# swarth100/dynfu

Hardware: AMD Instinct MI355X
Metric: frames/sec (warp-solve + TSDF fuse), 512^3 vol / 2k nodes / VGA depth (higher is better)
Workload: dtype f32; 1 GPU; C2: 512^3 TSDF, 640x480 depth, 2048 nodes, k=4, 262144 vertices, 5 GN x PCG<=256 (tol 1e-6), reference-parity energy (energy.t), lambda=200; parallelism=replicas x1 (one sequence per GPU, no collective), ranks_seen=1, repeats=5

## Files before the change

dynfu_amd/csrc/capi.cpp:

```cpp
#include <hip/hip_runtime.h>

#include <cmath>
#include <cstdarg>
#include <cstdio>
#include <cstring>
#include <map>
#include <mutex>
#include <new>
#include <utility>
#include <vector>

#include "../../include/dynfu_amd.h"
#include "kernels.hpp"
#include "dev_switch.hpp"
#include "solve.hpp"
#include "solve6.hpp"

namespace {

thread_local char g_err[512] = "";

int fail(int code, const char* fmt, ...) {
    va_list ap;
    va_start(ap, fmt);
// ... 87 lines not shown
    long cap_segs       = 0;
    hipError_t reserve(long nsegs) {
        if (nsegs <= cap_segs) return hipSuccess;
        (void)hipFree(seg_off), (void)hipFree(chunk_sums);
        seg_off = chunk_sums = nullptr, cap_segs = 0;
        hipError_t e;
        if ((e = hipMalloc((void**)&seg_off, sizeof(int32_t) * (size_t)(nsegs + 1))) != hipSuccess) return e;
        if ((e = hipMalloc((void**)&chunk_sums, sizeof(int32_t) * (size_t)dfa::mc_scan_chunks(nsegs))) != hipSuccess)
            return e;
        cap_segs = nsegs;
        return hipSuccess;
    }
};
struct McIndexedScratch {
    McScratch vert;
    int32_t* idx_off = nullptr;
    long cap_segs    = 0;
    hipError_t reserve(long nsegs) {
        hipError_t e = vert.reserve(nsegs);
        if (e != hipSuccess || nsegs <= cap_segs) return e;
        (void)hipFree(idx_off);
        idx_off = nullptr, cap_segs = 0;
        if ((e = hipMalloc((void**)&idx_off, sizeof(int32_t) * (size_t)(nsegs + 1))) != hipSuccess) return e;
        cap_segs = nsegs;
        return hipSuccess;
    }
};

bool want_grid(int D, long n_query) { return D >= 64 && ((long)D * n_query >= (1L << 22) || D >= 1024); }

}

struct dfa_solver {
    int max_D, max_N, k;
    size_t max_R;
    int ell_cap;
    dfa::SolveView v;
    dfa::SolveState* state;
    double* cost_partials;
    unsigned int* ticket;
    std::vector<void*> blocks;
    GridScratch grid;
    bool has_problem;
    bool timing;
    std::vector<hipEvent_t> events;
    std::vector<int> ev_pcg, ev_asm;
    size_t ev_used;
    int timed_solves = 0;
    dfa::MbGraphCache mb_graphs;
    dfa::TeamPcg team;
    bool deterministic = false;
    bool just_reset = false;
    bool graph_rows = false;
    long long* iters_total = nullptr;
    dfa_overlap_fn overlap_fn = nullptr;
    void* overlap_user        = nullptr;
    int* host_flag = nullptr;
};

struct dfa_solver6 {
    int max_D, max_N, k;
    dfa::Solve6View v;
    dfa::Solve6State* state;
    float* raw_w;
    int32_t* raw_reg;
    const float* node_dq;
    std::vector<void*> blocks;
    GridScratch grid;
    bool has_problem;
    std::map<int, hipGraphExec_t> pcg_graphs;
    int last_launches = 0;
    static constexpr int S6_RING = 4;
    int* mirror = nullptr;
    hipEvent_t done_ev[S6_RING] = {};
    int slot_gn[S6_RING] = {};
    unsigned long long solve_seq = 0, folded = 0;
    int pred[dfa::S6_HIST] = {};
    struct BudgetKey { int D, N, num_iter, gn_iter, linear_iter; float tol, tol_first, tol_decay, tol_adapt, gn_tol; } budget_key = {};
    bool graph_disabled = false;
    hipStream_t capture_stream = nullptr;
    bool timing = false;
    std::vector<hipEvent_t> events;
    size_t ev_used = 0;
    int pcg_key_D = -1;
};

namespace {
template <class T>
int plan6_alloc(dfa_solver6* s, T** out, size_t count) {
    void* p      = nullptr;
    hipError_t e = hipMalloc(&p, sizeof(T) * (count ? count : 1));
    if (e != hipSuccess) return hip_fail(e, "hipMalloc (solver6 plan)");
    s->blocks.push_back(p);
    *out = (T*)p;
    return DFA_OK;
}
}

namespace {
int timing_begin(dfa_solver* s, hipStream_t st) {
    if (s->ev_used + 2 > s->events.size()) {
        for (int i = 0; i < 2; ++i) {
            hipEvent_t e;
            if (hipEventCreate(&e) != hipSuccess) return -1;
            s->events.push_back(e);
        }
// ... 610 lines not shown
                                   out_normals, out_index, grid, S(stream)));
    return DFA_OK;
}

int dfa_correspond_projective(const float* vertices, const float* normals, int n, const float* vmap, int vmap_step,
                              const float* nmap, int nmap_step, int cols, int rows, float fx, float fy, float cx, float cy,
                              float dist_thresh, float min_cosine, float* out_vertices, float* out_normals,
                              int32_t* out_pixel, dfa_stream_t stream) {
    REQUIRE(n >= 0 && (n == 0 || vertices), "bad vertices");
    REQUIRE(vmap && cols > 0 && rows > 0 && vmap_step >= 16 * cols, "bad vertex map");
    REQUIRE(!nmap || nmap_step >= 16 * cols, "bad normal map pitch");
    REQUIRE(!out_normals || nmap, "normals requested without a normal map");
    REQUIRE(fx > 0.f && fy > 0.f && dist_thresh >= 0.f, "bad intrinsics / threshold");
    REQUIRE(((uintptr_t)vmap & 15) == 0 && (vmap_step & 15) == 0 && ((uintptr_t)nmap & 15) == 0 && (!nmap || (nmap_step & 15) == 0),
            "maps must be 16-byte aligned float4 images");
    HIP_TRY(dfa::launch_correspond_projective(vertices, normals, n, vmap, vmap_step, nmap, nmap_step, cols, rows, fx, fy, cx,
                                              cy, dist_thresh, min_cosine, out_vertices, out_normals, out_pixel,
                                              S(stream)));
    return DFA_OK;
}


int dfa_solver_create(int max_D, int max_N, int k, dfa_solver** out) {
    REQUIRE(out, "null out");
    *out = nullptr;
    REQUIRE(max_D > 0 && max_N >= 0, "bad sizes");
    REQUIRE(k >= 1 && k <= DFA_MAX_KNN, "k out of range 1..16");
    REQUIRE(max_D <= dfa::solve_pcg_max_nodes(), "more nodes than a plan supports (32768)");
    int ndev = 0;
    if (hipGetDeviceCount(&ndev) != hipSuccess || ndev == 0) return fail(DFA_ERR_NO_GPU, "no HIP device");
    dfa_solver* s = new (std::nothrow) dfa_solver();
    REQUIRE(s, "out of host memory");
    s->max_D = max_D, s->max_N = max_N, s->k = k;
    s->max_R       = (size_t)max_N + (size_t)max_D * k;
    s->ell_cap     = 256;
    s->has_problem = false;
    s->timing      = false;
    {
        const char* e    = getenv("DFA_ASSEMBLE_DETERMINISTIC");
        s->deterministic = e && atoi(e) != 0;
    }
    s->ev_used     = 0;
    std::memset(&s->v, 0, sizeof(s->v));
    const size_t R = s->max_R, D = (size_t)max_D;
    int rc = DFA_OK;
#define A(field, count) \
    if (rc == DFA_OK) rc = plan_alloc(s, &s->v.field, (count))
    A(ridx, R * k);
    A(rw, R * k);
    A(rtau, R);
    A(rb, R * 3);
    A(re, R * (size_t)dfa::solve_rec_words(k));
    A(reg_idx, D * k);
    A(blk_hist, D * (dfa::SOLVE_TG_BLOCKS + 1));
    A(node_ptr, D + 1);
    A(node_list, R * k);
    A(ell, D * s->ell_cap);
    A(ell_cnt, D);
    A(diag, D);
    A(g, D * 3);
    A(g_base, D * 3);
    A(t_base, D * 3);
    A(pk_perm, D);
    A(pk_perm2, D);
    A(pk_vals, D * s->ell_cap);
    A(pk_cols, D * s->ell_cap);
    A(mb_x, D);
    A(mb_r, D);
    A(mb_p, D);
    A(mb_s, D);
    A(mb_w, D);
    A(mb_u[0], D);
    A(mb_u[1], D);
    A(mb_m[0], D);
    A(mb_m[1], D);
    A(mb_t[0], D);
    A(mb_t[1], D);
    A(mb_gpart[0], (size_t)dfa::solve_mb_blocks(max_D));
    A(mb_gpart[1], (size_t)dfa::solve_mb_blocks(max_D));
    A(mb_dpart[0], (size_t)dfa::solve_mb_blocks(max_D));
    A(mb_dpart[1], (size_t)dfa::solve_mb_blocks(max_D));
    A(t, D * 3);
    A(huber, D);
    A(node_dq_out, D * 8);
#undef A
    if (rc == DFA_OK) {
        hipError_t e = s->grid.reserve(max_D);
        if (e != hipSuccess) rc = hip_fail(e, "hipMalloc (node grid)");
    }
    if (rc == DFA_OK && dfa::solve_team_pcg_fits(max_D) && (max_D > 2048 || dfa::kDevAB)) {
        s->v.team_stride = (max_D + 3) & ~3;
        rc = plan_alloc(s, &s->v.team_ctl, 1);
        const size_t areas = (size_t)3 * dfa::solve_team_pcg_rounds();
        if (rc == DFA_OK) rc = plan_alloc(s, &s->v.team_mt, areas * s->v.team_stride);
        if (rc == DFA_OK) rc = plan_alloc(s, &s->v.team_words, dfa::solve_team_pcg_words());
        if (rc == DFA_OK && (hipMemset(s->v.team_ctl, 0, sizeof(dfa::TeamCtl)) != hipSuccess ||
                             hipMemset(s->v.team_words, 0, sizeof(unsigned long long) * dfa::solve_team_pcg_words()) != hipSuccess ||
                             hipMemset(s->v.team_mt, 0, sizeof(float2) * areas * (size_t)s->v.team_stride) != hipSuccess))
            rc = fail(DFA_ERR_HIP, "hipMemset (team PCG)");
        if (rc == DFA_OK && hipHostMalloc((void**)&s->team.host_abort, sizeof(int), hipHostMallocDefault) == hipSuccess) {
            *s->team.host_abort = 0;
            s->team.ctl = s->v.team_ctl;
            if (const char* e0 = dfa::dev_env("DFA_MB_TEAM_EPOCH")) s->team.epoch = (unsigned)std::strtoul(e0, nullptr, 0);
        }
    }
    if (rc == DFA_OK) rc = plan_alloc(s, &s->state, 1);
    if (rc == DFA_OK) rc = plan_alloc(s, &s->iters_total, 1);
    if (rc == DFA_OK && hipMemset(s->iters_total, 0, sizeof(long long)) != hipSuccess) rc = DFA_ERR_HIP;
    if (rc == DFA_OK && hipHostMalloc((void**)&s->host_flag, 4 * sizeof(int), hipHostMallocDefault) != hipSuccess) s->host_flag = nullptr;
    if (rc == DFA_OK) rc = plan_alloc(s, &s->cost_partials, std::max<size_t>((R + 255) / 256 + 1, 1024) + 1024);
    if (rc == DFA_OK) rc = plan_alloc(s, &s->ticket, 64);
    if (rc == DFA_OK && hipMemset(s->ticket, 0, 64 * sizeof(unsigned int)) != hipSuccess)
        rc = fail(DFA_ERR_HIP, "hipMemset (ticket)");
    if (rc != DFA_OK) {
        dfa_solver_destroy(s);
        return rc;
    }
    *out = s;
    return DFA_OK;
}

void dfa_solver_destroy(dfa_solver* s) {
    if (!s) return;
    for (void* p : s->blocks) (void)hipFree(p);
    s->grid.release();
    for (hipEvent_t e : s->events) (void)hipEventDestroy(e);
    if (s->host_flag) (void)hipHostFree(s->host_flag);
    if (s->team.host_abort) (void)hipHostFree(s->team.host_abort);
    s->mb_graphs.release();
    delete s;
}

int dfa_solver_set_problem(dfa_solver* s, const float* node_pos, const float* node_dq, const float* node_w, int D,
                           const float* canon_vertices, const float* canon_normals, const float* live_vertices,
                           const float* live_normals, int N, dfa_stream_t stream) {
    (void)canon_normals;
    (void)live_normals;
    REQUIRE(s, "null plan");
    REQUIRE(node_pos && node_dq && node_w && D > 0, "no nodes");
    REQUIRE(N >= 0 && (N == 0 || (canon_vertices && live_vertices)), "bad vertex arrays");
    if (D > s->max_D || N > s->max_N)
        return fail(DFA_ERR_CAPACITY, "dfa_solver_set_problem: D=%d N=%d exceed the plan (max_D=%d max_N=%d)", D, N,
                    s->max_D, s->max_N);
    dfa::SolveView& v = s->v;
    v.N = N, v.D = D, v.k = s->k, v.Dpad = (D + 3) & ~3, v.ell_cap = s->ell_cap;
    v.deterministic = s->deterministic ? 1 : 0;
    v.node_pos = node_pos, v.node_dq = node_dq, v.node_w = node_w;
    v.canon = canon_vertices, v.live = live_vertices;
    hipStream_t st = S(stream);
    const dfa::KnnGridView* grid = nullptr;
    if (want_grid(D, (long)N + D) || dfa::dev_env_int("DFA_GRAPH_GRID", 0) != 0) {
        HIP_TRY(dfa::knn_grid_build(s->grid.v, node_pos, D, st));
        grid = &s->grid.v;
    }
    s->graph_rows = grid && dfa::solve_graph_rows_fits(v);
    if (s->graph_rows) {
        HIP_TRY(dfa::solve_build_graph_rows(v, *grid, s->state, s->ticket, 64, st));
    } else {
        if (N > 0) HIP_TRY(dfa::launch_knn(node_pos, node_w, D, canon_vertices, N, s->k, v.ridx, v.rw, grid, st));
        HIP_TRY(dfa::launch_knn(node_pos, node_w, D, node_pos, D, s->k, v.reg_idx, nullptr, grid, st));
        HIP_TRY(dfa::solve_build_graph(v, s->state, s->ticket, 64, st));
    }
    s->has_problem = true;
    s->just_reset  = true;
    return DFA_OK;
}

int dfa_solver_set_deterministic(dfa_solver* s, int on) {
    REQUIRE(s, "null plan");
    s->deterministic = on != 0;
    return DFA_OK;
}

int dfa_solver_solve(dfa_solver* s, const dfa_solve_params* p, dfa_stream_t stream) {
    REQUIRE(s && p, "null plan / params");
    REQUIRE(s->has_problem, "set_problem has not been called");
    REQUIRE(p->num_iter >= 0 && p->nonlinear_iter >= 0 && p->linear_iter >= 0, "negative iteration count");
    REQUIRE(p->tukey_offset > 0.f && p->psi_data > 0.f, "tukey_offset / psi_data must be positive");
    REQUIRE(p->lambda >= 0.f && std::isfinite(p->lambda), "lambda must be non-negative and finite");
    const dfa::SolveView& v = s->v;
    hipStream_t st          = S(stream);
    if (!s->just_reset) HIP_TRY(dfa::solve_reset(v, s->state, s->ticket, 64, st));
    s->just_reset = false;
    const double w_reg    = std::sqrt((double)p->lambda / ((double)v.D * (double)v.k));
    const float w_reg_f   = (float)w_reg;
    const float w_reg_sq  = w_reg_f * w_reg_f;
    if (s->timing) s->timed_solves += 1;
    if (s->host_flag) s->host_flag[0] = s->host_flag[1] = 0;
    s->mb_graphs.call = 0;
    int not_launched = 0;
    int gn_launched = 0;
    bool huber_done = false;
    const bool big_budget = (long)p->num_iter * p->nonlinear_iter > 8;
    const bool pcg_async  = dfa::solve_pcg_is_async(v, &s->team, p->linear_iter);
    const bool no_regradient = dfa::dev_env("DFA_NO_REGRADIENT") != nullptr;
    for (int outer = 0; outer < p->num_iter; ++outer) {
        if (s->host_flag && s->host_flag[1] == 2) s->host_flag[1] = 0;
        int gn_in_outer = 0;
        for (int gn = 0; gn < p->nonlinear_iter; ++gn) {
            if (big_budget && gn_in_outer >= 4 && gn_in_outer % 4 == 0 && s->host_flag && !s->host_flag[1] && pcg_async) {
                HIP_TRY(hipMemcpyAsync(&s->host_flag[1], &s->state->converged, sizeof(int), hipMemcpyDeviceToHost, st));
                HIP_TRY(hipStreamSynchronize(st));
            }
            if (s->host_flag && s->host_flag[1]) {
                ++not_launched;
                continue;
            }
            ++gn_in_outer;
            if (gn > 0 && p->gn_tol == 0.f && p->lambda > 0.f && !no_regradient) {
                int evg = s->timing ? timing_begin(s, st) : -1;
                HIP_TRY(dfa::solve_regradient(v, s->state, st));
                timing_end(s, evg, st);
                if (evg >= 0) s->ev_asm.push_back(evg);
                if (s->overlap_fn) s->overlap_fn(s->overlap_user, stream, gn_launched);
                ++gn_launched;
// ... 111 lines not shown
    }
    out->pcg_launches      = (int)s->ev_pcg.size();
    out->assemble_launches = (int)s->ev_asm.size();
    out->solves            = s->timed_solves;
    if (s->iters_total) HIP_TRY(hipMemcpy(&out->pcg_iters, s->iters_total, sizeof(long long), hipMemcpyDeviceToHost));
    if (s->has_problem && s->v.D > 0) {
        std::vector<int32_t> cnt((size_t)s->v.D);
        HIP_TRY(hipMemcpy(cnt.data(), s->v.ell_cnt, sizeof(int32_t) * cnt.size(), hipMemcpyDeviceToHost));
        long long nnz = 0;
        for (int32_t c : cnt) nnz += c;
        out->matrix_nnz = nnz;
    }
    return DFA_OK;
}


int dfa_compute_points_normals(const uint16_t* depth, int depth_step, int cols, int rows, float fx, float fy, float cx,
                               float cy, float* points, int points_step, float* normals, int normals_step,
                               dfa_stream_t stream) {
    REQUIRE(depth && points && normals && cols > 0 && rows > 0, "bad images");
    REQUIRE(depth_step >= cols * 2 && points_step >= cols * 16 && normals_step >= cols * 16, "row step smaller than a row");
    REQUIRE(fx != 0.f && fy != 0.f, "zero focal length");
    HIP_TRY(dfa::launch_points_normals(depth, depth_step, cols, rows, fx, fy, cx, cy, points, points_step, normals,
                                       normals_step, S(stream)));
    return DFA_OK;
}

int dfa_solver6_create(int max_D, int max_N, int k, dfa_solver6** out) {
    REQUIRE(out, "null out");
    *out = nullptr;
    REQUIRE(max_D > 0 && max_N >= 0, "bad sizes");
    REQUIRE(k >= 1 && k <= 8, "k out of range 1..8");
    int ndev = 0;
    if (hipGetDeviceCount(&ndev) != hipSuccess || ndev == 0) return fail(DFA_ERR_NO_GPU, "no HIP device");
    dfa_solver6* s = new (std::nothrow) dfa_solver6();
    REQUIRE(s, "out of host memory");
    s->max_D = max_D, s->max_N = max_N, s->k = k, s->has_problem = false, s->node_dq = nullptr;
    std::memset(&s->v, 0, sizeof(s->v));
    s->v.cap = DFA_SOLVE6_ROW_BLOCKS;
    const size_t N = (size_t)max_N, D = (size_t)max_D, cap = (size_t)s->v.cap;
    int rc = DFA_OK;
#define A(field, count) \
    if (rc == DFA_OK) rc = plan6_alloc(s, &s->v.field, (count))
    A(idx, N * k);
    A(wn, N * k);
    A(idx_nat, N * k);
    A(near, N);
    A(vptr, D + 1);
    A(vlist, N);
    A(vperm, N);
    A(canon_own, N * 3);
    A(canon_n_own, N * 3);
    A(reg_idx, D * k);
    A(blk_hist, D * (dfa::SOLVE_TG_BLOCKS + 1));
    A(node_ptr, D + 1);
    A(node_list, N * k + 1);
    A(rnode_ptr, D + 1);
    A(rnode_list, D * k + 1);
    A(dq, D * 8);
    A(dq_prev, D * 8);
    A(ghat, D * 3);
    A(rec, N * (12 + (k <= 4 ? 4 : 8)));
    A(cost_part, (N + 255) / 256 + (D * k + 255) / 256 + 1);
    A(valid_part, (N + 255) / 256 + (D * k + 255) / 256 + 1);
    A(mnode, D * 48);
    A(rho, N);
    A(rres, D * k * 3);
    A(rvec, D * k * 18);
    A(rhub, D * k);
    A(bcols, D * cap);
    A(bcnt, D);
    A(bfu, D);
    A(rslot, D * cap);
    A(utab, D * 256);
    A(eslot, N * k * k);
    A(pair_list, N * k * k);
    A(pair_ptr, D * (cap + 1));
    A(bvals, D * cap * 36);
    A(minv, D * 36);
    A(g, D * 6);
    A(x, D * 6);
    A(r, D * 6);
    A(p, D * 6);
    A(s, D * 6);
    A(w, D * 6);
    A(u[0], D * 6);
    A(u[1], D * 6);
    A(t[0], D * 6);
    A(t[1], D * 6);
    A(m[0], D * 6);
    A(m[1], D * 6);
    A(g_part[0], (size_t)dfa::s6_matvec_blocks(max_D));
    A(g_part[1], (size_t)dfa::s6_matvec_blocks(max_D));
    A(d_part[0], (size_t)dfa::s6_matvec_blocks(max_D));
    A(d_part[1], (size_t)dfa::s6_matvec_blocks(max_D));
#undef A
    if (rc == DFA_OK) rc = plan6_alloc(s, &s->raw_w, N * k);
    if (rc == DFA_OK) rc = plan6_alloc(s, &s->raw_reg, D * (k + 1));
    if (rc == DFA_OK) rc = plan6_alloc(s, &s->state, 1);
    if (rc == DFA_OK) {
        bool ok = hipHostMalloc((void**)&s->mirror, dfa_solver6::S6_RING * dfa::S6_HIST * sizeof(int), hipHostMallocDefault) == hipSuccess;
        for (int i = 0; ok && i < dfa_solver6::S6_RING; ++i)
            ok = hipEventCreateWithFlags(&s->done_ev[i], hipEventDisableTiming) == hipSuccess;
        if (ok) {
            std::memset(s->mirror, 0, dfa_solver6::S6_RING * dfa::S6_HIST * sizeof(int));
        } else {
            (void)hipGetLastError();
// ... 274 lines not shown
```

dynfu_amd/csrc/solve.hip:

```cpp
#include <hip/hip_runtime.h>
#include <cstring>

#include <algorithm>
#include <map>
#include <mutex>

#include <float.h>

#include "dq_device.hpp"
#include "dev_switch.hpp"
#include "kernels.hpp"
#include "knn_device.hpp"
#include "pcg_rules.hpp"
#include "solve.hpp"

namespace dfa {


constexpr int TG_BLOCKS = SOLVE_TG_BLOCKS;

__global__ __launch_bounds__(1024) void tg_count_kernel(const int32_t* __restrict__ ridx, size_t total, int D,
                                                        int32_t* __restrict__ blk_hist ) {
    extern __shared__ int32_t hist[];
    for (int i = threadIdx.x; i < D; i += blockDim.x) hist[i] = 0;
    __syncthreads();
    const size_t chunk = (total + TG_BLOCKS - 1) / TG_BLOCKS;
    const size_t beg = chunk * blockIdx.x, end = min(beg + chunk, total);
    for (size_t e = beg + threadIdx.x; e < end; e += blockDim.x) {
        const int n = ridx[e];
        if (n >= 0) atomicAdd(&hist[n], 1);
    }
    __syncthreads();
    for (int i = threadIdx.x; i < D; i += blockDim.x) blk_hist[(size_t)blockIdx.x * D + i] = hist[i];
}

__global__ __launch_bounds__(256) void tg_colscan_kernel(int32_t* __restrict__ blk_hist , int D) {
    const int i = blockIdx.x * blockDim.x + threadIdx.x;
    if (i >= D) return;
    constexpr int G = 32;
    static_assert(TG_BLOCKS % G == 0, "workgroups of the counting sort in groups");
    int run = 0;
    for (int b0 = 0; b0 < TG_BLOCKS; b0 += G) {
        int h[G];
#pragma unroll
        for (int b = 0; b < G; ++b) h[b] = blk_hist[(size_t)(b0 + b) * D + i];
#pragma unroll
        for (int b = 0; b < G; ++b) {
            blk_hist[(size_t)(b0 + b) * D + i] = run;
            run += h[b];
        }
    }
    blk_hist[(size_t)TG_BLOCKS * D + i] = run;
}

__global__ __launch_bounds__(1024) void tg_fill_kernel(const int32_t* __restrict__ ridx, size_t total, int D,
                                                       const int32_t* __restrict__ blk_base ,
                                                       int32_t* __restrict__ node_ptr, uint32_t* __restrict__ node_list) {
    extern __shared__ int32_t cursor[];
    __shared__ int32_t wave_tot[16];
    __shared__ int32_t carry_sh;
    const int lane = threadIdx.x & 63, wave = threadIdx.x >> 6;
    if (threadIdx.x == 0) carry_sh = 0;
    __syncthreads();
    for (int base = 0; base < D; base += 1024) {
        const int i = base + threadIdx.x;
        const int v = i < D ? blk_base[(size_t)TG_BLOCKS * D + i] : 0;
        const int incl = wave_inclusive_scan(v);
        if (lane == 63) wave_tot[wave] = incl;
        __syncthreads();
        int off = carry_sh + incl - v;
        for (int w = 0; w < wave; ++w) off += wave_tot[w];
        if (i < D) {
            cursor[i] = off + blk_base[(size_t)blockIdx.x * D + i];
            if (blockIdx.x == 0) node_ptr[i] = off;
        }
        __syncthreads();
        if (threadIdx.x == 1023) carry_sh = off + v;
        __syncthreads();
    }
    if (blockIdx.x == 0 && threadIdx.x == 0) node_ptr[D] = carry_sh;
    const size_t chunk = (total + TG_BLOCKS - 1) / TG_BLOCKS;
    const size_t beg = chunk * blockIdx.x, end = min(beg + chunk, total);
    for (size_t e = beg + threadIdx.x; e < end; e += blockDim.x) {
        const int n = ridx[e];
        if (n >= 0) node_list[atomicAdd(&cursor[n], 1)] = (uint32_t)e;
    }
}


template <int K>
__device__ __forceinline__ void load_row_graph(const SolveView& s, size_t r, int (&n)[K], float (&w)[K]) {
    if (s.k == K) {
#pragma unroll
        for (int q = 0; q < K / 4; ++q) {
            const int4 iv   = reinterpret_cast<const int4*>(s.ridx + r * K)[q];
            const float4 wv = reinterpret_cast<const float4*>(s.rw + r * K)[q];
            n[4 * q] = iv.x, n[4 * q + 1] = iv.y, n[4 * q + 2] = iv.z, n[4 * q + 3] = iv.w;
            w[4 * q] = wv.x, w[4 * q + 1] = wv.y, w[4 * q + 2] = wv.z, w[4 * q + 3] = wv.w;
        }
    } else {
#pragma unroll
        for (int j = 0; j < K; ++j) n[j] = j < s.k ? s.ridx[r * s.k + j] : -1, w[j] = j < s.k ? s.rw[r * s.k + j] : 0.f;
    }
}

template <int K>
__device__ __forceinline__ float tukey_weight(const SolveView& s, size_t v, float tukey_offset, float psi_data) {
    const f3 c = mk3(s.canon[3 * v], s.canon[3 * v + 1], s.canon[3 * v + 2]);
    DQ sum     = dq_identity();
    int n[K];
    float w[K];
    load_row_graph<K>(s, v, n, w);
#pragma unroll
    for (int h = 0; h < K; h += 4) {
        float tx[4], ty[4], tz[4];
        DQ q[4];
#pragma unroll
        for (int jj = 0; jj < 4; ++jj) {
            const int nn = n[h + jj] >= 0 ? n[h + jj] : 0;
            tx[jj] = s.t[3 * nn], ty[jj] = s.t[3 * nn + 1], tz[jj] = s.t[3 * nn + 2];
            q[jj]  = dq_load(s.node_dq + 8 * (size_t)nn);
        }
#pragma unroll
        for (int jj = 0; jj < 4; ++jj) {
            if (n[h + jj] >= 0) {
                const DQ cur = dq_mul(dq_from_translation(tx[jj], ty[jj], tz[jj]), q[jj]);
                sum          = dq_mul(sum, dq_scale(cur, w[h + jj]));
            }
        }
    }
    const f3 warped = dq_transform(dq_normalize(sum), c);
    const float ex = s.live[3 * v] - warped.x, ey = s.live[3 * v + 1] - warped.y, ez = s.live[3 * v + 2] - warped.z;
    const float d = sqrtf(ex * ex + ey * ey + ez * ez) / tukey_offset;
    if (d < psi_data) {
// ... 211 lines not shown
    if (m >= 0 && m != n) ids[0] = m, ws[0] = -1.f, ids[1] = n, ws[1] = +1.f;
}

template <int K>
__device__ __forceinline__ void store_row_graph(const SolveView& s, size_t r, const int (&ids)[K], const float (&ws)[K]) {
#pragma unroll
    for (int q = 0; q < K / 4; ++q) {
        reinterpret_cast<int4*>(s.ridx + r * K)[q]  = make_int4(ids[4 * q], ids[4 * q + 1], ids[4 * q + 2], ids[4 * q + 3]);
        reinterpret_cast<float4*>(s.rw + r * K)[q] = make_float4(ws[4 * q], ws[4 * q + 1], ws[4 * q + 2], ws[4 * q + 3]);
    }
}

template <int K>
__global__ __launch_bounds__(256) void prepare_rows_kernel(SolveView s, SolveState* __restrict__ st,
                                                           unsigned int* __restrict__ ticket, int nticket) {
    const size_t R = (size_t)s.N + (size_t)s.D * s.k;
    const size_t r = (size_t)blockIdx.x * blockDim.x + threadIdx.x;
    if (r < (size_t)3 * s.D) s.t[r] = 0.f;
    if (blockIdx.x == 0) {
        unsigned int* w = (unsigned int*)st;
        for (int j = threadIdx.x; j < (int)(sizeof(SolveState) / 4); j += blockDim.x) w[j] = 0u;
        for (int j = threadIdx.x; j < nticket; j += blockDim.x) ticket[j] = 0u;
    }
    if (r >= R) return;
    const int k = s.k;
    int ids[K];
    float ws[K];
    const bool wide = k == K && K % 4 == 0;
    if (r < (size_t)s.N) {
#pragma unroll
        for (int c = 0; c < 3; ++c) s.rb[3 * r + c] = s.live[3 * r + c] - s.canon[3 * r + c];
        if (wide) load_row_graph<K>(s, r, ids, ws);
        else {
#pragma unroll
            for (int j = 0; j < K; ++j)
                if (j < k) ids[j] = s.ridx[r * k + j], ws[j] = s.rw[r * k + j];
        }
    } else {
        const int e = (int)(r - (size_t)s.N), n = e / k, m = s.reg_idx[e];
        reg_row_slots<K>(m, n, ids, ws);
        if (wide) store_row_graph<K>(s, r, ids, ws);
        else {
#pragma unroll
            for (int j = 0; j < K; ++j)
                if (j < k) s.ridx[r * k + j] = ids[j], s.rw[r * k + j] = ws[j];
        }
        s.rb[3 * r + 0] = s.rb[3 * r + 1] = s.rb[3 * r + 2] = 0.f;
    }
    store_record_head<K>(s, r, ids, ws, wide);
}

template <int K>
__global__ __launch_bounds__(256) void graph_rows_kernel(SolveView s, KnnGridView grid, SolveState* __restrict__ st,
                                                         unsigned int* __restrict__ ticket, int nticket, int data_blocks) {
    static_assert(K % 4 == 0, "rows by 16-byte stores");
    if ((int)blockIdx.x < data_blocks) {
        const int v = blockIdx.x * blockDim.x + threadIdx.x;
        if (v >= s.N) return;
        const f3 q = mk3(s.canon[3 * (size_t)v], s.canon[3 * (size_t)v + 1], s.canon[3 * (size_t)v + 2]);
        KnnList<K> best;
        knn_grid_query<K>(*grid.desc, grid.cell_start, grid.sorted, q, best);
        int ids[K];
        float ws[K];
        knn_ids_weights<K>(best, K, s.node_pos, s.node_w, true, q, ids, ws);
        const size_t r = (size_t)v;
        store_row_graph<K>(s, r, ids, ws);
        s.rb[3 * r + 0] = s.live[3 * r + 0] - q.x, s.rb[3 * r + 1] = s.live[3 * r + 1] - q.y, s.rb[3 * r + 2] = s.live[3 * r + 2] - q.z;
        store_record_head<K>(s, r, ids, ws, true);
        return;
    }
    const int b = (int)blockIdx.x - data_blocks;
    const int i = b * (int)blockDim.x + (int)threadIdx.x;
    if (i < 3 * s.D) s.t[i] = 0.f;
    if (b == 0) {
        unsigned int* w = (unsigned int*)st;
        for (int j = threadIdx.x; j < (int)(sizeof(SolveState) / 4); j += blockDim.x) w[j] = 0u;
        for (int j = threadIdx.x; j < nticket; j += blockDim.x) ticket[j] = 0u;
    }
    const int n = b * 4 + (int)(threadIdx.x >> 6), lane = threadIdx.x & 63;
    if (n >= s.D) return;
    const f3 q = mk3(s.node_pos[3 * (size_t)n], s.node_pos[3 * (size_t)n + 1], s.node_pos[3 * (size_t)n + 2]);
    int near[K];
    knn_wave_search<K>(*grid.desc, grid.cell_start, grid.sorted, q, lane, near);
    if (lane >= K) return;
    int m = -1;
#pragma unroll
    for (int j = 0; j < K; ++j)
        if (j == lane) m = near[j];
    const size_t e = (size_t)n * K + lane, r = (size_t)s.N + e;
    s.reg_idx[e] = m;
    int ids[K];
    float ws[K];
    reg_row_slots<K>(m, n, ids, ws);
    store_row_graph<K>(s, r, ids, ws);
    s.rb[3 * r + 0] = s.rb[3 * r + 1] = s.rb[3 * r + 2] = 0.f;
    store_record_head<K>(s, r, ids, ws, true);
}


constexpr int HASH      = 512;
constexpr int HASH_MASK = HASH - 1;

struct FixedScale {
    float up;
    double down;
};
__device__ __forceinline__ FixedScale solve_fixed_scale(float amax) {
    int e = 0;
    (void)frexpf(fmaxf(amax, 1e-30f), &e);
    e = e < -80 ? -80 : e > 100 ? 100 : e;
    FixedScale f;
    f.up   = ldexpf(1.f, 40 - e);
    f.down = ldexp(1.0, e - 40);
    return f;
}
__device__ __forceinline__ FixedScale fixed_scale_for_rows(FixedScale f, int rows) {
    const int extra = 32 - __clz((unsigned)max(rows, 1) >> 22);
    if (extra > 0) f.up = ldexpf(f.up, -extra), f.down = ldexp(f.down, extra);
    return f;
}
__device__ __forceinline__ void fixed_add(long long* cell, float v, float up) {
    const float x  = truncf(fabsf(v) * up);
    const float hf = floorf(x * 2.3283064365386963e-10f);
    const uint32_t hi = (uint32_t)hf, lo = (uint32_t)fmaf(hf, -4294967296.f, x);
    atomicAdd(reinterpret_cast<unsigned long long*>(v < 0.f ? cell + HASH : cell), ((unsigned long long)hi << 32) | lo);
}

template <int K>
__device__ __forceinline__ float4 load_record(const SolveView& s, size_t r, int (&idx)[K], float (&w)[K]) {
    const float* rec = s.re + r * (size_t)solve_rec_words(s.k);
    if (s.k == K && (K % 8) == 0) {
        const float4* v = (const float4*)rec;
#pragma unroll
        for (int q = 0; q < K / 8; ++q) {
            const float4 i4 = v[q];
            const uint32_t u[4] = {__float_as_uint(i4.x), __float_as_uint(i4.y), __float_as_uint(i4.z), __float_as_uint(i4.w)};
#pragma unroll
            for (int h = 0; h < 4; ++h) {
                const int lo = (int)(u[h] & 0xffffu), hi = (int)(u[h] >> 16);
                idx[8 * q + 2 * h]     = lo == 0xffff ? -1 : lo;
                idx[8 * q + 2 * h + 1] = hi == 0xffff ? -1 : hi;
            }
        }
#pragma unroll
        for (int q = 0; q < K / 4; ++q) {
            const float4 w4 = v[K / 8 + q];
            w[4 * q] = w4.x, w[4 * q + 1] = w4.y, w[4 * q + 2] = w4.z, w[4 * q + 3] = w4.w;
        }
        return v[K / 8 + K / 4];
// ... 877 lines not shown
            for (int i = 0; i < NT / 64; ++i) gamma += red0[i], delta += red1[i];
            PROF_MARK(1);
            if (!(gamma > target)) break;
            const float beta  = cg_beta(it == 0, gamma, gamma_old);
            const float denom = cg_denom(it == 0, gamma, delta, beta, alpha_old);
            if (!(denom > 0.f)) break;
            const float alpha = gamma / denom;
#pragma unroll
            for (int j = 0; j < P; ++j)
#pragma unroll
                for (int c = 0; c < NC; ++c) {
                    cg_update_row(alpha, beta, uA[j][c], wA[j][c], pA[j][c], sA[j][c], xA[j][c], rA_[j][c]);
                    cg_update_row(alpha, beta, uB[j][c], wB[j][c], pB[j][c], sB[j][c], xB[j][c], rB_[j][c]);
                    uA[j][c]  = minvA[j] * rA_[j][c];
                    uB[j][c]  = minvB[j] * rB_[j][c];
                }
            ++it;
            gamma_old = gamma, alpha_old = alpha;
            PROF_MARK(2);
            publish(uA, uB);
            __syncthreads();
            PROF_MARK(4);
        }
    }
#ifdef DFA_PCG_PROFILE
    if (tid == 0 && c0 == 0)
        for (int i = 0; i < 6; ++i) st->prof[i] += pc_[i];
#endif
#pragma unroll
    for (int j = 0; j < P; ++j)
#pragma unroll
        for (int c = 0; c < NC; ++c) {
            if (rowA[j] >= 0) s.t[3 * rowA[j] + c0 + c] += xA[j][c];
            if (rowB[j] >= 0) s.t[3 * rowB[j] + c0 + c] += xB[j][c];
        }
    if (tid == 0) {
        if (NC == 3) pcg_book_launch(st, rz0, it, false);
        else pcg_book_launch_of_three(st, rz0, it, false);
    }
}


#define KDISPATCH(kernel, k, ...)                      \
    do {                                               \
        if ((k) <= 4) kernel<4> __VA_ARGS__;           \
        else if ((k) <= 8) kernel<8> __VA_ARGS__;      \
        else kernel<16> __VA_ARGS__;                   \
    } while (0)

hipError_t solve_transpose_graph(const int32_t* ridx, size_t total, int D, int32_t* blk_hist, int32_t* node_ptr,
                                 uint32_t* node_list, hipStream_t st) {
    const size_t lds = sizeof(int32_t) * (size_t)D;
    tg_count_kernel<<<TG_BLOCKS, 1024, lds, st>>>(ridx, total, D, blk_hist);
    tg_colscan_kernel<<<(D + 255) / 256, 256, 0, st>>>(blk_hist, D);
    tg_fill_kernel<<<TG_BLOCKS, 1024, lds, st>>>(ridx, total, D, blk_hist, node_ptr, node_list);
    return hipGetLastError();
}

static hipError_t transpose_rows(const SolveView& s, hipStream_t st) {
    const int D = s.D, k = s.k;
    const size_t total = ((size_t)s.N + (size_t)D * k) * k;
    const size_t lds = sizeof(int32_t) * (size_t)D;
    tg_count_kernel<<<TG_BLOCKS, 1024, lds, st>>>(s.ridx, total, D, s.blk_hist);
    tg_colscan_kernel<<<(D + 255) / 256, 256, 0, st>>>(s.blk_hist, D);
    tg_fill_kernel<<<TG_BLOCKS, 1024, lds, st>>>(s.ridx, total, D, s.blk_hist, s.node_ptr, s.node_list);
    if (s.deterministic) sort_node_lists_kernel<<<D, 256, 0, st>>>(s.node_ptr, s.node_list);
    return hipGetLastError();
}

hipError_t solve_build_graph(const SolveView& s, SolveState* state, unsigned int* ticket, int nticket, hipStream_t st) {
    const int D = s.D, N = s.N, k = s.k;
    const size_t R = (size_t)N + (size_t)D * k;
    const size_t threads = R > (size_t)3 * D ? R : (size_t)3 * D;
    KDISPATCH(prepare_rows_kernel, k, <<<(unsigned)((threads + 255) / 256), 256, 0, st>>>(s, state, ticket, nticket));
    return transpose_rows(s, st);
}

bool solve_graph_rows_fits(const SolveView& s) {
    const int k = s.k;
    return s.N > 0 && (k == 4 || k == 8 || k == 16) &&
           ((reinterpret_cast<uintptr_t>(s.ridx) | reinterpret_cast<uintptr_t>(s.rw) | reinterpret_cast<uintptr_t>(s.re)) & 15u) == 0 &&
           dev_env_int("DFA_GRAPH_ROWS", 1) != 0;
}

hipError_t solve_build_graph_rows(const SolveView& s, const KnnGridView& grid, SolveState* state, unsigned int* ticket,
                                  int nticket, hipStream_t st) {
    const int data_blocks = (s.N + 255) / 256, reg_blocks = (s.D + 3) / 4;
    KDISPATCH(graph_rows_kernel, s.k, <<<data_blocks + reg_blocks, 256, 0, st>>>(s, grid, state, ticket, nticket, data_blocks));
    return transpose_rows(s, st);
}

int solve_residual_blocks(const SolveView& s) {
    const size_t R  = (size_t)s.N + (size_t)s.D * s.k;
    const size_t nb = (R + 255) / 256;
    return (int)(nb < (size_t)LIN_MAX_BLOCKS ? nb : (size_t)LIN_MAX_BLOCKS);
}

hipError_t solve_linearise(const SolveView& s, SolveState* state, double* cost_partials, unsigned int* ticket,
                           int update_weights, int mode, float gn_tol, float tukey_offset, float psi_data,
                           float w_reg_sq, float huber_psi, long long* iters_total, hipStream_t st) {
    const int nb = solve_residual_blocks(s);
    LineariseArgs a{update_weights, mode, gn_tol, tukey_offset, psi_data, w_reg_sq, iters_total, huber_psi};
    KDISPATCH(linearise_kernel, s.k, <<<nb, 256, 0, st>>>(s, state, cost_partials, ticket, a));
    return hipGetLastError();
}

hipError_t solve_reset(const SolveView& s, SolveState* state, unsigned int* ticket, int nticket, hipStream_t st) {
    reset_kernel<<<(3 * s.D + 255) / 256, 256, 0, st>>>(s.t, 3 * s.D, state, ticket, nticket);
    return hipGetLastError();
}

hipError_t solve_huber(const SolveView& s, float psi_reg, hipStream_t st) {
    huber_kernel<<<(s.D + 255) / 256, 256, 0, st>>>(s, psi_reg);
    return hipGetLastError();
}

hipError_t solve_assemble(const SolveView& s, SolveState* state, int save_base, float w_reg_sq, hipStream_t st) {
    const float amax_unset = std::max(1.0f, w_reg_sq);
    if (s.deterministic) KDISPATCH(assemble_det_kernel, s.k, <<<s.D, 256, 0, st>>>(s, state, save_base, amax_unset));
    else KDISPATCH(assemble_kernel, s.k, <<<s.D, 256, 0, st>>>(s, state, save_base, amax_unset));
    return hipGetLastError();
}

__global__ __launch_bounds__(256) void regradient_kernel(SolveView s, SolveState* __restrict__ st) {
    if (st->done || st->converged) return;
    const int a = blockIdx.x * blockDim.x + threadIdx.x;
    if (a == 0) st->cost_stale = 1, st->weights_fresh = 0;
    if (a >= s.D) return;
    const int cnt = s.ell_cnt[a];
    float sx = 0.f, sy = 0.f, sz = 0.f;
    for (int q = 0; q < cnt; ++q) {
        const float2 e = s.ell[(size_t)q * s.D + a];
        const int col  = __float_as_int(e.y);
        sx = fmaf(e.x, s.t[3 * col] - s.t_base[3 * col], sx);
        sy = fmaf(e.x, s.t[3 * col + 1] - s.t_base[3 * col + 1], sy);
        sz = fmaf(e.x, s.t[3 * col + 2] - s.t_base[3 * col + 2], sz);
    }
    s.g[3 * a] = s.g_base[3 * a] - sx, s.g[3 * a + 1] = s.g_base[3 * a + 1] - sy, s.g[3 * a + 2] = s.g_base[3 * a + 2] - sz;
}

hipError_t solve_regradient(const SolveView& s, SolveState* state, hipStream_t st) {
    regradient_kernel<<<(s.D + 255) / 256, 256, 0, st>>>(s, state);
// ... 757 lines not shown
```

dynfu_amd/csrc/solve.hpp:

```cpp
#pragma once
#include <hip/hip_runtime.h>
#include <stdint.h>

#include "kernels.hpp"

namespace dfa {

struct SolveState {
    double initial_cost;
    double cost;
    double final_cost;
    double grad_first;
    int have_initial;
    int done;
    int gn_iters;
    int pcg_iters;
    int max_row_nnz;
    int overflow;
    int pcg_fallback;
    int split_iters;
    unsigned int split_ticket;
    int mb_done;
    int converged;
    int mb_skip, mb_iters;
    int weights_fresh;
    int gn_noop;
    int cost_stale;
    float mb_rz0, mb_gamma_prev[2], mb_alpha_prev[2];
    float amax;
    long long prof[8];
};

__host__ __device__ inline bool solve_rec_ids16(int k) { return k % 8 == 0; }
__host__ __device__ inline int solve_rec_words(int k) { return solve_rec_ids16(k) ? k + k / 2 + 4 : 2 * k + 4; }
__host__ __device__ inline int solve_rec_tail(int k) { return solve_rec_words(k) - 4; }

__device__ __forceinline__ void solve_mark_at_floor(SolveState* st) {
    if (st->weights_fresh) st->converged = 1;
    else if (!st->converged) st->converged = 2;
}

struct TeamCtl {
    unsigned int count[3];
    unsigned int abort[3];
    unsigned int finished[3];
    int iters[3];
    float rz0[3];
    unsigned int at_floor[3];
};

struct SolveView {
    int N, D, k, Dpad, ell_cap;
    int deterministic;
    const float* node_pos;
    const float* node_dq;
    const float* node_w;
    const float* canon;
    const float* live;
    int32_t* ridx;
    float* rw;
    float* rtau;
    float* rb;
    float* re;
    int32_t* reg_idx;
    int32_t* blk_hist;
    int32_t* node_ptr;
    uint32_t* node_list;
    float2* ell;
    int32_t* ell_cnt;
    float* diag;
    float* g;
    float* g_base;
    float* t_base;
    int32_t* pk_perm;
    int32_t* pk_perm2;
    float* pk_vals;
    uint16_t* pk_cols;
    float4 *mb_x, *mb_r, *mb_p, *mb_s, *mb_w, *mb_u[2], *mb_m[2], *mb_t[2];
    float *mb_gpart[2], *mb_dpart[2];
    TeamCtl* team_ctl;
    float2* team_mt;
    unsigned long long* team_words;
    int team_stride;
    float* t;
    float* huber;
    float* node_dq_out;
};

constexpr int SOLVE_TG_BLOCKS = 256;
hipError_t solve_build_graph(const SolveView& s, SolveState* state, unsigned int* ticket, int nticket, hipStream_t st);
bool solve_graph_rows_fits(const SolveView& s);
hipError_t solve_build_graph_rows(const SolveView& s, const KnnGridView& grid, SolveState* state, unsigned int* ticket,
                                  int nticket, hipStream_t st);
hipError_t solve_transpose_graph(const int32_t* ridx, size_t total, int D, int32_t* blk_hist, int32_t* node_ptr,
                                 uint32_t* node_list, hipStream_t st);
int solve_residual_blocks(const SolveView& s);
hipError_t solve_linearise(const SolveView& s, SolveState* state, double* cost_partials, unsigned int* ticket,
                           int update_weights, int mode, float gn_tol, float tukey_offset, float psi_data,
                           float w_reg_sq, float huber_psi ,
                           long long* iters_total , hipStream_t st);
hipError_t solve_huber(const SolveView& s, float psi_reg, hipStream_t st);
hipError_t solve_reset(const SolveView& s, SolveState* state, unsigned int* ticket, int nticket, hipStream_t st);
hipError_t solve_assemble(const SolveView& s, SolveState* state, int save_base , float w_reg_sq,
                          hipStream_t st);
hipError_t solve_regradient(const SolveView& s, SolveState* state, hipStream_t st);
int solve_pcg_max_nodes();
__host__ __device__ inline int solve_mb_rows_per_block() { return 16; }
__host__ __device__ inline int solve_mb_blocks(int D) { return (D + 15) / 16; }
struct MbGraphCache {
    struct Entry {
        int it0 = 0, it1 = 0;
        float tol = 0.f;
        SolveView view;
        const SolveState* state = nullptr;
        hipGraphExec_t exec = nullptr;
    };
    Entry e[24];
    int used = 0;
// ... 26 lines not shown
```

Before: 1636 frames/s.

## Fuse transpose counting into graph-row build and fold column scan into fill

The per-chunk node histogram is now accumulated inside graph_rows_kernel through an LDS hash tally flushed with global atomics, so the separate tg_count_kernel pass is skipped on the grid path. The column prefix scan moves into tg_fill_kernel, which removes the tg_colscan launch. Two double-buffered histogram tables let each fill pass zero the table for the next problem instead of a separate memset. This trades two launches and an extra read of ridx for LDS hashing, global atomics and a redundant per-block column scan inside the fill kernel.

```diff
diff --git a/dynfu_amd/csrc/capi.cpp b/dynfu_amd/csrc/capi.cpp
--- a/dynfu_amd/csrc/capi.cpp
+++ b/dynfu_amd/csrc/capi.cpp
@@ -163,6 +163,10 @@
     bool deterministic = false;
     bool just_reset = false;
     bool graph_rows = false;
+    int32_t* blk_tab[2] = {nullptr, nullptr};
+    size_t blk_dirty[2] = {0, 0};
+    int blk_cur         = 0;
+    bool blk_known      = true;
     long long* iters_total = nullptr;
     dfa_overlap_fn overlap_fn = nullptr;
     void* overlap_user        = nullptr;
@@ -879,7 +883,6 @@
     A(rb, R * 3);
     A(re, R * (size_t)dfa::solve_rec_words(k));
     A(reg_idx, D * k);
-    A(blk_hist, D * (dfa::SOLVE_TG_BLOCKS + 1));
     A(node_ptr, D + 1);
     A(node_list, R * k);
     A(ell, D * s->ell_cap);
@@ -911,6 +914,11 @@
     A(huber, D);
     A(node_dq_out, D * 8);
 #undef A
+    for (int i = 0; i < 2 && rc == DFA_OK; ++i) {
+        rc = plan_alloc(s, &s->blk_tab[i], D * dfa::SOLVE_TG_BLOCKS);
+        if (rc == DFA_OK && hipMemset(s->blk_tab[i], 0, sizeof(int32_t) * D * dfa::SOLVE_TG_BLOCKS) != hipSuccess)
+            rc = fail(DFA_ERR_HIP, "hipMemset (transposition tables)");
+    }
     if (rc == DFA_OK) {
         hipError_t e = s->grid.reserve(max_D);
         if (e != hipSuccess) rc = hip_fail(e, "hipMalloc (node grid)");
@@ -975,6 +983,14 @@
     v.node_pos = node_pos, v.node_dq = node_dq, v.node_w = node_w;
     v.canon = canon_vertices, v.live = live_vertices;
     hipStream_t st = S(stream);
+    const size_t tab_words = (size_t)D * dfa::SOLVE_TG_BLOCKS;
+    if (!s->blk_known) {
+        for (int i = 0; i < 2; ++i) HIP_TRY(hipMemsetAsync(s->blk_tab[i], 0, sizeof(int32_t) * (size_t)s->max_D * dfa::SOLVE_TG_BLOCKS, st));
+        s->blk_dirty[0] = s->blk_dirty[1] = 0;
+    }
+    s->blk_known = false;
+    const int cur = s->blk_cur;
+    v.blk_hist = s->blk_tab[cur], v.blk_clear = s->blk_tab[cur ^ 1], v.blk_clear_words = s->blk_dirty[cur ^ 1];
     const dfa::KnnGridView* grid = nullptr;
     if (want_grid(D, (long)N + D) || dfa::dev_env_int("DFA_GRAPH_GRID", 0) != 0) {
         HIP_TRY(dfa::knn_grid_build(s->grid.v, node_pos, D, st));
@@ -988,6 +1004,7 @@
         HIP_TRY(dfa::launch_knn(node_pos, node_w, D, node_pos, D, s->k, v.reg_idx, nullptr, grid, st));
         HIP_TRY(dfa::solve_build_graph(v, s->state, s->ticket, 64, st));
     }
+    s->blk_dirty[cur] = tab_words, s->blk_dirty[cur ^ 1] = 0, s->blk_cur = cur ^ 1, s->blk_known = true;
     s->has_problem = true;
     s->just_reset  = true;
     return DFA_OK;
@@ -1205,7 +1222,7 @@
     A(canon_own, N * 3);
     A(canon_n_own, N * 3);
     A(reg_idx, D * k);
-    A(blk_hist, D * (dfa::SOLVE_TG_BLOCKS + 1));
+    A(blk_hist, D * dfa::SOLVE_TG_BLOCKS);
     A(node_ptr, D + 1);
     A(node_list, N * k + 1);
     A(rnode_ptr, D + 1);
diff --git a/dynfu_amd/csrc/solve.hip b/dynfu_amd/csrc/solve.hip
--- a/dynfu_amd/csrc/solve.hip
+++ b/dynfu_amd/csrc/solve.hip
@@ -19,12 +19,14 @@
 
 constexpr int TG_BLOCKS = SOLVE_TG_BLOCKS;
 
+__host__ __device__ __forceinline__ size_t tg_chunk_entries(size_t total) { return (total + TG_BLOCKS - 1) / TG_BLOCKS; }
+
 __global__ __launch_bounds__(1024) void tg_count_kernel(const int32_t* __restrict__ ridx, size_t total, int D,
                                                         int32_t* __restrict__ blk_hist ) {
     extern __shared__ int32_t hist[];
     for (int i = threadIdx.x; i < D; i += blockDim.x) hist[i] = 0;
     __syncthreads();
-    const size_t chunk = (total + TG_BLOCKS - 1) / TG_BLOCKS;
+    const size_t chunk = tg_chunk_entries(total);
     const size_t beg = chunk * blockIdx.x, end = min(beg + chunk, total);
     for (size_t e = beg + threadIdx.x; e < end; e += blockDim.x) {
         const int n = ridx[e];
@@ -34,44 +36,85 @@
     for (int i = threadIdx.x; i < D; i += blockDim.x) blk_hist[(size_t)blockIdx.x * D + i] = hist[i];
 }
 
-__global__ __launch_bounds__(256) void tg_colscan_kernel(int32_t* __restrict__ blk_hist , int D) {
-    const int i = blockIdx.x * blockDim.x + threadIdx.x;
-    if (i >= D) return;
-    constexpr int G = 32;
-    static_assert(TG_BLOCKS % G == 0, "workgroups of the counting sort in groups");
-    int run = 0;
-    for (int b0 = 0; b0 < TG_BLOCKS; b0 += G) {
-        int h[G];
-#pragma unroll
-        for (int b = 0; b < G; ++b) h[b] = blk_hist[(size_t)(b0 + b) * D + i];
-#pragma unroll
-        for (int b = 0; b < G; ++b) {
-            blk_hist[(size_t)(b0 + b) * D + i] = run;
-            run += h[b];
-        }
-    }
-    blk_hist[(size_t)TG_BLOCKS * D + i] = run;
+struct TgTally {
+    int* key;
+    int* cnt;
+};
+template <int SLOTS>
+__device__ __forceinline__ void tg_tally_reset(const TgTally& t) {
+    for (int h = threadIdx.x; h < SLOTS; h += blockDim.x) t.key[h] = -1, t.cnt[h] = 0;
+}
+template <int SLOTS>
+__device__ __forceinline__ void tg_tally_add(const TgTally& t, int key) {
+    static_assert((SLOTS & (SLOTS - 1)) == 0, "a power of two");
+    unsigned h = ((unsigned)key * 2654435761u) >> (32 - __builtin_ctz((unsigned)SLOTS));
+    for (;;) {
+        int cur = t.key[h];
+        if (cur == -1) cur = atomicCAS(&t.key[h], -1, key);
+        if (cur == -1 || cur == key) break;
+        h = (h + 1) & (unsigned)(SLOTS - 1);
+    }
+    atomicAdd(&t.cnt[h], 1);
+}
+template <int K, int SLOTS>
+__device__ __forceinline__ void tg_tally_row(const TgTally& t, unsigned r, const int (&ids)[K], unsigned chunk, unsigned first_chunk, int D) {
+    const unsigned e0 = r * (unsigned)K;
+    unsigned c = e0 / chunk, left = chunk - (e0 - c * chunk);
+#pragma unroll
+    for (int j = 0; j < K; ++j) {
+        while ((unsigned)j >= left) ++c, left += chunk;
+        if (ids[j] >= 0) tg_tally_add<SLOTS>(t, (int)(c - first_chunk) * D + ids[j]);
+    }
+}
+template <int SLOTS>
+__device__ __forceinline__ void tg_tally_flush(const TgTally& t, unsigned first_chunk, int D, int32_t* __restrict__ blk_hist) {
+    for (int h = threadIdx.x; h < SLOTS; h += blockDim.x) {
+        const int key = t.key[h];
+        if (key < 0) continue;
+        const int c = key / D, n = key - c * D;
+        __hip_atomic_fetch_add(&blk_hist[(size_t)(first_chunk + (unsigned)c) * D + n], t.cnt[h], __ATOMIC_RELAXED, __HIP_MEMORY_SCOPE_AGENT);
+    }
 }
 
 __global__ __launch_bounds__(1024) void tg_fill_kernel(const int32_t* __restrict__ ridx, size_t total, int D,
-                                                       const int32_t* __restrict__ blk_base ,
-                                                       int32_t* __restrict__ node_ptr, uint32_t* __restrict__ node_list) {
+                                                       const int32_t* __restrict__ blk_hist ,
+                                                       int32_t* __restrict__ node_ptr, uint32_t* __restrict__ node_list,
+                                                       int32_t* __restrict__ blk_clear, size_t blk_clear_words) {
     extern __shared__ int32_t cursor[];
     __shared__ int32_t wave_tot[16];
     __shared__ int32_t carry_sh;
     const int lane = threadIdx.x & 63, wave = threadIdx.x >> 6;
+    {
+        const size_t share = (blk_clear_words + TG_BLOCKS - 1) / TG_BLOCKS;
+        const size_t cb = share * blockIdx.x, ce = min(cb + share, blk_clear_words);
+        for (size_t w = cb + threadIdx.x; w < ce; w += blockDim.x) blk_clear[w] = 0;
+    }
     if (threadIdx.x == 0) carry_sh = 0;
     __syncthreads();
+    constexpr int G = 32;
+    static_assert(TG_BLOCKS % G == 0, "workgroups of the counting sort in groups");
     for (int base = 0; base < D; base += 1024) {
         const int i = base + threadIdx.x;
-        const int v = i < D ? blk_base[(size_t)TG_BLOCKS * D + i] : 0;
+        int v = 0, mine = 0;
+        if (i < D) {
+            for (int b0 = 0; b0 < TG_BLOCKS; b0 += G) {
+                int h[G];
+#pragma unroll
+                for (int b = 0; b < G; ++b) h[b] = blk_hist[(size_t)(b0 + b) * D + i];
+#pragma unroll
+                for (int b = 0; b < G; ++b) {
+                    if (b0 + b == (int)blockIdx.x) mine = v;
+                    v += h[b];
+                }
+            }
+        }
         const int incl = wave_inclusive_scan(v);
         if (lane == 63) wave_tot[wave] = incl;
         __syncthreads();
         int off = carry_sh + incl - v;
         for (int w = 0; w < wave; ++w) off += wave_tot[w];
         if (i < D) {
-            cursor[i] = off + blk_base[(size_t)blockIdx.x * D + i];
+            cursor[i] = off + mine;
             if (blockIdx.x == 0) node_ptr[i] = off;
         }
         __syncthreads();
@@ -79,7 +122,7 @@
         __syncthreads();
     }
     if (blockIdx.x == 0 && threadIdx.x == 0) node_ptr[D] = carry_sh;
-    const size_t chunk = (total + TG_BLOCKS - 1) / TG_BLOCKS;
+    const size_t chunk = tg_chunk_entries(total);
     const size_t beg = chunk * blockIdx.x, end = min(beg + chunk, total);
     for (size_t e = beg + threadIdx.x; e < end; e += blockDim.x) {
         const int n = ridx[e];
@@ -397,49 +440,66 @@
 
 template <int K>
 __global__ __launch_bounds__(256) void graph_rows_kernel(SolveView s, KnnGridView grid, SolveState* __restrict__ st,
-                                                         unsigned int* __restrict__ ticket, int nticket, int data_blocks) {
+                                                         unsigned int* __restrict__ ticket, int nticket, int data_blocks,
+                                                         unsigned tg_chunk) {
     static_assert(K % 4 == 0, "rows by 16-byte stores");
+    constexpr int SLOTS = 256 * K;
+    static_assert(4 * K <= 256, "a regularisation workgroup's rows fit the tally");
+    __shared__ int tally_key[SLOTS], tally_cnt[SLOTS];
+    const TgTally tally{tally_key, tally_cnt};
+    tg_tally_reset<SLOTS>(tally);
+    __syncthreads();
+    unsigned first_chunk;
     if ((int)blockIdx.x < data_blocks) {
+        first_chunk = blockIdx.x * blockDim.x * (unsigned)K / tg_chunk;
         const int v = blockIdx.x * blockDim.x + threadIdx.x;
-        if (v >= s.N) return;
-        const f3 q = mk3(s.canon[3 * (size_t)v], s.canon[3 * (size_t)v + 1], s.canon[3 * (size_t)v + 2]);
-        KnnList<K> best;
-        knn_grid_query<K>(*grid.desc, grid.cell_start, grid.sorted, q, best);
-        int ids[K];
-        float ws[K];
-        knn_ids_weights<K>(best, K, s.node_pos, s.node_w, true, q, ids, ws);
-        const size_t r = (size_t)v;
-        store_row_graph<K>(s, r, ids, ws);
-        s.rb[3 * r + 0] = s.live[3 * r + 0] - q.x, s.rb[3 * r + 1] = s.live[3 * r + 1] - q.y, s.rb[3 * r + 2] = s.live[3 * r + 2] - q.z;
-        store_record_head<K>(s, r, ids, ws, true);
-        return;
-    }
-    const int b = (int)blockIdx.x - data_blocks;
-    const int i = b * (int)blockDim.x + (int)threadIdx.x;
-    if (i < 3 * s.D) s.t[i] = 0.f;
-    if (b == 0) {
-        unsigned int* w = (unsigned int*)st;
-        for (int j = threadIdx.x; j < (int)(sizeof(SolveState) / 4); j += blockDim.x) w[j] = 0u;
-        for (int j = threadIdx.x; j < nticket; j += blockDim.x) ticket[j] = 0u;
-    }
-    const int n = b * 4 + (int)(threadIdx.x >> 6), lane = threadIdx.x & 63;
-    if (n >= s.D) return;
-    const f3 q = mk3(s.node_pos[3 * (size_t)n], s.node_pos[3 * (size_t)n + 1], s.node_pos[3 * (size_t)n + 2]);
-    int near[K];
-    knn_wave_search<K>(*grid.desc, grid.cell_start, grid.sorted, q, lane, near);
-    if (lane >= K) return;
-    int m = -1;
-#pragma unroll
-    for (int j = 0; j < K; ++j)
-        if (j == lane) m = near[j];
-    const size_t e = (size_t)n * K + lane, r = (size_t)s.N + e;
-    s.reg_idx[e] = m;
-    int ids[K];
-    float ws[K];
-    reg_row_slots<K>(m, n, ids, ws);
-    store_row_graph<K>(s, r, ids, ws);
-    s.rb[3 * r + 0] = s.rb[3 * r + 1] = s.rb[3 * r + 2] = 0.f;
-    store_record_head<K>(s, r, ids, ws, true);
+        if (v < s.N) {
+            const f3 q = mk3(s.canon[3 * (size_t)v], s.canon[3 * (size_t)v + 1], s.canon[3 * (size_t)v + 2]);
+            KnnList<K> best;
+            knn_grid_query<K>(*grid.desc, grid.cell_start, grid.sorted, q, best);
+            int ids[K];
+            float ws[K];
+            knn_ids_weights<K>(best, K, s.node_pos, s.node_w, true, q, ids, ws);
+            const size_t r = (size_t)v;
+            store_row_graph<K>(s, r, ids, ws);
+            s.rb[3 * r + 0] = s.live[3 * r + 0] - q.x, s.rb[3 * r + 1] = s.live[3 * r + 1] - q.y, s.rb[3 * r + 2] = s.live[3 * r + 2] - q.z;
+            store_record_head<K>(s, r, ids, ws, true);
+            tg_tally_row<K, SLOTS>(tally, (unsigned)v, ids, tg_chunk, first_chunk, s.D);
+        }
+    } else {
+        const int b = (int)blockIdx.x - data_blocks;
+        first_chunk = ((unsigned)s.N + (unsigned)b * 4u * K) * (unsigned)K / tg_chunk;
+        const int i = b * (int)blockDim.x + (int)threadIdx.x;
+        if (i < 3 * s.D) s.t[i] = 0.f;
+        if (b == 0) {
+            unsigned int* w = (unsigned int*)st;
+            for (int j = threadIdx.x; j < (int)(sizeof(SolveState) / 4); j += blockDim.x) w[j] = 0u;
+            for (int j = threadIdx.x; j < nticket; j += blockDim.x) ticket[j] = 0u;
+        }
+        const int n = b * 4 + (int)(threadIdx.x >> 6), lane = threadIdx.x & 63;
+        if (n < s.D) {
+            const f3 q = mk3(s.node_pos[3 * (size_t)n], s.node_pos[3 * (size_t)n + 1], s.node_pos[3 * (size_t)n + 2]);
+            int near[K];
+            knn_wave_search<K>(*grid.desc, grid.cell_start, grid.sorted, q, lane, near);
+            if (lane < K) {
+                int m = -1;
+#pragma unroll
+                for (int j = 0; j < K; ++j)
+                    if (j == lane) m = near[j];
+                const size_t e = (size_t)n * K + lane, r = (size_t)s.N + e;
+                s.reg_idx[e] = m;
+                int ids[K];
+                float ws[K];
+                reg_row_slots<K>(m, n, ids, ws);
+                store_row_graph<K>(s, r, ids, ws);
+                s.rb[3 * r + 0] = s.rb[3 * r + 1] = s.rb[3 * r + 2] = 0.f;
+                store_record_head<K>(s, r, ids, ws, true);
+                tg_tally_row<K, SLOTS>(tally, (unsigned)r, ids, tg_chunk, first_chunk, s.D);
+            }
+        }
+    }
+    __syncthreads();
+    tg_tally_flush<SLOTS>(tally, first_chunk, s.D, s.blk_hist);
 }
 
 
@@ -1423,18 +1483,18 @@
                                  uint32_t* node_list, hipStream_t st) {
     const size_t lds = sizeof(int32_t) * (size_t)D;
     tg_count_kernel<<<TG_BLOCKS, 1024, lds, st>>>(ridx, total, D, blk_hist);
-    tg_colscan_kernel<<<(D + 255) / 256, 256, 0, st>>>(blk_hist, D);
-    tg_fill_kernel<<<TG_BLOCKS, 1024, lds, st>>>(ridx, total, D, blk_hist, node_ptr, node_list);
+    tg_fill_kernel<<<TG_BLOCKS, 1024, lds, st>>>(ridx, total, D, blk_hist, node_ptr, node_list, nullptr, 0);
     return hipGetLastError();
 }
 
-static hipError_t transpose_rows(const SolveView& s, hipStream_t st) {
-    const int D = s.D, k = s.k;
-    const size_t total = ((size_t)s.N + (size_t)D * k) * k;
+static size_t transpose_entries(const SolveView& s) { return ((size_t)s.N + (size_t)s.D * s.k) * s.k; }
+
+static hipError_t transpose_rows(const SolveView& s, bool counted, hipStream_t st) {
+    const int D = s.D;
+    const size_t total = transpose_entries(s);
     const size_t lds = sizeof(int32_t) * (size_t)D;
-    tg_count_kernel<<<TG_BLOCKS, 1024, lds, st>>>(s.ridx, total, D, s.blk_hist);
-    tg_colscan_kernel<<<(D + 255) / 256, 256, 0, st>>>(s.blk_hist, D);
-    tg_fill_kernel<<<TG_BLOCKS, 1024, lds, st>>>(s.ridx, total, D, s.blk_hist, s.node_ptr, s.node_list);
+    if (!counted) tg_count_kernel<<<TG_BLOCKS, 1024, lds, st>>>(s.ridx, total, D, s.blk_hist);
+    tg_fill_kernel<<<TG_BLOCKS, 1024, lds, st>>>(s.ridx, total, D, s.blk_hist, s.node_ptr, s.node_list, s.blk_clear, s.blk_clear_words);
     if (s.deterministic) sort_node_lists_kernel<<<D, 256, 0, st>>>(s.node_ptr, s.node_list);
     return hipGetLastError();
 }
@@ -1444,7 +1504,7 @@
     const size_t R = (size_t)N + (size_t)D * k;
     const size_t threads = R > (size_t)3 * D ? R : (size_t)3 * D;
     KDISPATCH(prepare_rows_kernel, k, <<<(unsigned)((threads + 255) / 256), 256, 0, st>>>(s, state, ticket, nticket));
-    return transpose_rows(s, st);
+    return transpose_rows(s, false, st);
 }
 
 bool solve_graph_rows_fits(const SolveView& s) {
@@ -1457,8 +1517,9 @@
 hipError_t solve_build_graph_rows(const SolveView& s, const KnnGridView& grid, SolveState* state, unsigned int* ticket,
                                   int nticket, hipStream_t st) {
     const int data_blocks = (s.N + 255) / 256, reg_blocks = (s.D + 3) / 4;
-    KDISPATCH(graph_rows_kernel, s.k, <<<data_blocks + reg_blocks, 256, 0, st>>>(s, grid, state, ticket, nticket, data_blocks));
-    return transpose_rows(s, st);
+    const unsigned tg_chunk = (unsigned)tg_chunk_entries(transpose_entries(s));
+    KDISPATCH(graph_rows_kernel, s.k, <<<data_blocks + reg_blocks, 256, 0, st>>>(s, grid, state, ticket, nticket, data_blocks, tg_chunk));
+    return transpose_rows(s, true, st);
 }
 
 int solve_residual_blocks(const SolveView& s) {
diff --git a/dynfu_amd/csrc/solve.hpp b/dynfu_amd/csrc/solve.hpp
--- a/dynfu_amd/csrc/solve.hpp
+++ b/dynfu_amd/csrc/solve.hpp
@@ -64,6 +64,8 @@
     float* re;
     int32_t* reg_idx;
     int32_t* blk_hist;
+    int32_t* blk_clear;
+    size_t blk_clear_words;
     int32_t* node_ptr;
     uint32_t* node_list;
     float2* ell;
```

Result: slower. 1538 frames/s (-6.0%).
